# 10183308/popsift

Measured on AMD Instinct MI355X. Metric: Mpix/s SIFT extract on 1920x1080 (keypoints+descriptors), higher is better.
Workload: dtype f32; 1 GPU; 1920x1080 u8 grayscale, default popsift::Config (2x upscale, 9 octaves, 3 levels, PopSift mode, loop descriptor, RootSift); distinct_images_per_gpu=16, contexts_per_gpu=3, images_per_launch=16

## Files before the change

### include/popsift_hip.h

```cpp
#ifndef POPSIFT_HIP_H
#define POPSIFT_HIP_H

#include <stddef.h>
#include <stdint.h>

#ifdef __cplusplus
extern "C" {
#endif

#define POPSIFT_HIP_MAX_OCTAVES 20
#define POPSIFT_HIP_MAX_LEVELS 12
#define POPSIFT_HIP_MAX_BATCH 16
#define POPSIFT_HIP_GAUSS_ALIGN 32
#define POPSIFT_HIP_ORI_MAX 4

typedef enum popsift_hip_status {
    POPSIFT_HIP_OK = 0,
    POPSIFT_HIP_ERR_INVALID = -1,
    POPSIFT_HIP_ERR_DEVICE = -2,
    POPSIFT_HIP_ERR_NO_DEVICE = -3,
    POPSIFT_HIP_ERR_OOM = -4,
    POPSIFT_HIP_ERR_STATE = -5,
    POPSIFT_HIP_ERR_TOO_SMALL = -6
} popsift_hip_status;
// ... 189 lines not shown
    int32_t reserved;
} popsift_hip_match_opts;
typedef struct popsift_hip_pair {
    int32_t l, r;
    float   dist_best, dist_second;
} popsift_hip_pair;
void popsift_hip_default_match_opts(popsift_hip_match_opts* opts);
int  popsift_hip_match_pairs(const popsift_hip_devfeatures* l, const popsift_hip_devfeatures* r,
                             const popsift_hip_match_opts* opts, popsift_hip_pair* pairs, size_t cap, int* n_pairs);

typedef struct popsift_hip_bytefeatures popsift_hip_bytefeatures;
int popsift_hip_bytefeatures_from_host(int device, const uint8_t* desc, int n_descriptors, popsift_hip_bytefeatures** out);
int popsift_hip_bytefeatures_from_set(const popsift_hip_devfeatures* f, popsift_hip_bytefeatures** out);
int popsift_hip_clone_results_u8(popsift_hip_ctx* ctx, int k, popsift_hip_bytefeatures** out);
int popsift_hip_bytefeatures_free(popsift_hip_bytefeatures* f);
int popsift_hip_bytefeatures_info(const popsift_hip_bytefeatures* f, int* device, int* n_descriptors);
int popsift_hip_bytefeatures_download(const popsift_hip_bytefeatures* f, uint8_t* desc, int32_t* rev);
int popsift_hip_match_bytes(const popsift_hip_bytefeatures* l, const popsift_hip_bytefeatures* r, popsift_hip_match* out);
int popsift_hip_match_pairs_bytes(const popsift_hip_bytefeatures* l, const popsift_hip_bytefeatures* r,
                                  const popsift_hip_match_opts* opts, popsift_hip_pair* pairs, size_t cap, int* n_pairs);

int popsift_hip_get_report(const popsift_hip_ctx* ctx, popsift_hip_report* rep);
int popsift_hip_set_profile(popsift_hip_ctx* ctx, int profile);

int popsift_hip_octave_dims(const popsift_hip_ctx* ctx, int octave, int* w, int* h);
int popsift_hip_download_plane(popsift_hip_ctx* ctx, int octave, int kind, int level, float* out);
int popsift_hip_upload_plane(popsift_hip_ctx* ctx, int octave, int kind, int level, const float* in);
int popsift_hip_download_extrema(popsift_hip_ctx* ctx, popsift_hip_extremum* out, size_t cap, int* n);
int popsift_hip_rerun_keypoint_stages(popsift_hip_ctx* ctx);
enum { POPSIFT_HIP_DEBUG_DET_QCAP = 1, POPSIFT_HIP_DEBUG_CAND_CAP = 2, POPSIFT_HIP_DEBUG_OHIST_CAP = 3,
       POPSIFT_HIP_DEBUG_FAIL_ALLOC = 4, POPSIFT_HIP_DEBUG_DESC_ROWS = 5,
       POPSIFT_HIP_DEBUG_KP_WAVES = 7, POPSIFT_HIP_DEBUG_BLUR_PATH = 8, POPSIFT_HIP_DEBUG_BLUR_SEG = 9,
       POPSIFT_HIP_DEBUG_PYR_TAIL = 10, POPSIFT_HIP_DEBUG_DIRECT_PATH = 11,
       POPSIFT_HIP_DEBUG_DESC_CAP = 12, POPSIFT_HIP_DEBUG_SCALE_PATH = 13 };
int popsift_hip_debug_set(popsift_hip_ctx* ctx, int what, int value);

#ifdef __cplusplus
}
#endif
#endif
```

### popsift_amd/_capi.py

```python
import ctypes as C
import os

import numpy as np

_HERE = os.path.dirname(os.path.abspath(__file__))
LIB_PATH = os.environ.get("POPSIFT_HIP_LIB") or os.path.join(_HERE, "libpopsift_hip.so")

MAX_OCTAVES = 20
ORI_MAX = 4

OK = 0
ERR_INVALID, ERR_DEVICE, ERR_NO_DEVICE, ERR_OOM, ERR_STATE, ERR_TOO_SMALL = -1, -2, -3, -4, -5, -6

SIFT_POPSIFT, SIFT_OPENCV, SIFT_VLFEAT = 0, 1, 2
GAUSS_VLFEAT_COMPUTE, GAUSS_VLFEAT_RELATIVE, GAUSS_VLFEAT_RELATIVE_ALL = 0, 1, 2
GAUSS_OPENCV_COMPUTE, GAUSS_FIXED9, GAUSS_FIXED15 = 3, 4, 5
DESC_LOOP, DESC_ILOOP, DESC_GRID, DESC_IGRID, DESC_NOTILE = 0, 1, 2, 3, 4
NORM_ROOTSIFT, NORM_CLASSIC = 0, 1
SCALE_DEFAULT, SCALE_DIRECT = 0, 1


class Params(C.Structure):
    _fields_ = [
        ("octaves", C.c_int32), ("levels", C.c_int32), ("sigma", C.c_float),
# ... 94 lines not shown
    ("popsift_hip_devfeatures_free", C.c_int, [_vp]),
    ("popsift_hip_devfeatures_info", C.c_int, [_vp, _ip, _ip, _ip]),
    ("popsift_hip_devfeatures_ptrs", C.c_int, [_vp, C.POINTER(_vp), C.POINTER(_vp), C.POINTER(_vp)]),
    ("popsift_hip_devfeatures_alloc", C.c_int, [C.c_int, C.c_int, C.c_int, C.POINTER(_vp)]),
    ("popsift_hip_devfeatures_from_host", C.c_int, [C.c_int, _vp, C.c_int, C.POINTER(_vp)]),
    ("popsift_hip_devfeatures_download", C.c_int, [_vp, _vp, _vp]),
    ("popsift_hip_devfeatures_download_u8", C.c_int, [_vp, _vp]),
    ("popsift_hip_match_sets", C.c_int, [_vp, _vp, _vp]),
    ("popsift_hip_match_set_path", C.c_int, [C.c_int]),
    ("popsift_hip_default_match_opts", None, [C.POINTER(MatchOpts)]),
    ("popsift_hip_match_pairs", C.c_int, [_vp, _vp, C.POINTER(MatchOpts), _vp, C.c_size_t, _ip]),
    ("popsift_hip_bytefeatures_from_host", C.c_int, [C.c_int, _vp, C.c_int, C.POINTER(_vp)]),
    ("popsift_hip_bytefeatures_from_set", C.c_int, [_vp, C.POINTER(_vp)]),
    ("popsift_hip_clone_results_u8", C.c_int, [_vp, C.c_int, C.POINTER(_vp)]),
    ("popsift_hip_bytefeatures_free", C.c_int, [_vp]),
    ("popsift_hip_bytefeatures_info", C.c_int, [_vp, _ip, _ip]),
    ("popsift_hip_bytefeatures_download", C.c_int, [_vp, _vp, _vp]),
    ("popsift_hip_match_bytes", C.c_int, [_vp, _vp, _vp]),
    ("popsift_hip_match_pairs_bytes", C.c_int, [_vp, _vp, C.POINTER(MatchOpts), _vp, C.c_size_t, _ip]),
    ("popsift_hip_get_report", C.c_int, [_vp, C.POINTER(Report)]),
    ("popsift_hip_set_profile", C.c_int, [_vp, C.c_int]),
    ("popsift_hip_octave_dims", C.c_int, [_vp, C.c_int, _ip, _ip]),
    ("popsift_hip_download_plane", C.c_int, [_vp, C.c_int, C.c_int, C.c_int, _vp]),
    ("popsift_hip_upload_plane", C.c_int, [_vp, C.c_int, C.c_int, C.c_int, _vp]),
    ("popsift_hip_download_extrema", C.c_int, [_vp, _vp, C.c_size_t, _ip]),
    ("popsift_hip_rerun_keypoint_stages", C.c_int, [_vp]),
    ("popsift_hip_debug_set", C.c_int, [_vp, C.c_int, C.c_int]),
]
MATCH_AUTO, MATCH_EXACT, MATCH_SCREEN = 0, 1, 2
STAGES = ("pyramid", "detect", "refine", "orientation", "scan", "descriptor")
DEBUG_DET_QCAP, DEBUG_CAND_CAP, DEBUG_OHIST_CAP, DEBUG_FAIL_ALLOC, DEBUG_DESC_ROWS, DEBUG_KP_WAVES = 1, 2, 3, 4, 5, 7
DEBUG_BLUR_PATH, DEBUG_BLUR_SEG, DEBUG_PYR_TAIL, DEBUG_DIRECT_PATH, DEBUG_DESC_CAP = 8, 9, 10, 11, 12
DEBUG_SCALE_PATH = 13
MAX_BATCH = 16
IMG_HOST_U8, IMG_HOST_F32, IMG_DEV_U8, IMG_DEV_F32, IMG_PINNED_U8, IMG_PINNED_F32 = range(6)

_lib = None


def _desc_type(fmt):
    if fmt == "f32":
        return np.float32
    if fmt == "u8":
        return np.uint8
    raise ValueError("fmt: 'f32' or 'u8', got %r" % (fmt,))


def quantize_u8(desc):
    d = np.asarray(desc, np.float32)
    with np.errstate(invalid="ignore"):
        pos = d > 0
        t = np.trunc(d)
        r = np.where(np.abs(d - t) >= np.float32(0.5), t + np.float32(1.0), t)
        r = np.where(d >= np.float32(255.0), np.float32(255.0), r)
        r = np.where(pos, r, np.float32(0.0))
    return r.astype(np.uint8)


class PopsiftHipError(RuntimeError):
    def __init__(self, status, where, detail=""):
        self.status = status
        msg = "%s failed: %d (%s)" % (where, status, lib().popsift_hip_strerror(status).decode())
        if detail:
            msg += ": " + detail
        super().__init__(msg)

# ... 448 lines not shown
```

### popsift_amd/csrc/ctx.hip

```cpp
#include <hip/hip_runtime.h>

#include <algorithm>
#include <atomic>
#include <cmath>
#include <cstdarg>
#include <cstddef>
#include <cstdio>
#include <cstdlib>
#include <cstring>
#include <new>
#include <type_traits>
#include <vector>

#include "devfeatures.h"
#include "kernels.h"
#include "sift_types.h"
#include "trace.h"

using namespace popsift_hip;

namespace {

constexpr int PITCH_ALIGN = 64;
constexpr int PROFILE_REPS = 4;
// ... 72 lines not shown
};

struct popsift_hip_ctx {
    int                device = 0;
    popsift_hip_params p{};
    int                levels = 3, L = 6;
    GaussRows<POPSIFT_HIP_MAX_LEVELS> tab{};
    GaussRows<POPSIFT_HIP_MAX_LEVELS> abs0{};
    float*             d_abs0 = nullptr;
    int                direct_path = 0;
    GaussRows<POPSIFT_HIP_MAX_OCTAVES> dd{};
    float*             d_dd = nullptr;
    int                scale_path = 0;
    SiftConsts         sc{};
    hipStream_t        stream = nullptr;
    hipEvent_t         ev_begin = nullptr, ev_end = nullptr;
    hipEvent_t         ev_stage[POPSIFT_HIP_STAGE_COUNT + 1] = {};

    int  in_w = 0, in_h = 0;
    int  frozen_octaves = -1;
    bool have_image = false, finished = false;
    bool batch_ok = false;
    int  nb = 1;
    bool describe = false;
    int  ori_given = 0;
    int  frames_max = 0;

    ImageSlot slot[PS_MAX_BATCH];
    BatchDesc bd{};
    PyrDesc   pd{};
    int       kp_waves = 65536;
    int       det_qcap = 1 << 30;
    int       desc_rows = 1 << 30;
    BlurTune  blur_tune{0, 0};
    int       pyr_tail = 0;
    int       cand_cap_init = 1 << 20;
    bool      cand_cap_user = false;
    int       ohist_cap_init = 0;
    int       desc_cap_init = 0;
    size_t    ext_cap = 0;
    int       cand_cap = 0, desc_cap = 0;
    size_t    ohist_cap = 0;
    hipStream_t copy_stream = nullptr;
    hipEvent_t  ev_u8 = nullptr;
    bool     copy_pending = false;
    unsigned long submit_seq = 0, copy_seq = 0;
    Counters* d_ct = nullptr;
    Counters* h_ct = nullptr;
    PyrDesc*  d_pd = nullptr;
    PyrDesc*  h_pd = nullptr;
    int       n_feat[PS_MAX_BATCH] = {}, n_desc[PS_MAX_BATCH] = {};

    int                    fail_alloc_in = 0;
    int                    profile = 0;
    std::vector<EventPair> blur_events;
    size_t                 blur_events_used = 0;
    popsift_hip_report     rep{};

    char err[256] = {0};
};

namespace {

int fail(popsift_hip_ctx* c, int code, const char* fmt, ...)
{
    if (c) {
// ... 78 lines not shown
    auto& a0 = c->abs0;
    memset(&a0, 0, sizeof(a0));
    if (p.gauss_mode == POPSIFT_HIP_GAUSS_VLFEAT_RELATIVE_ALL) {
        for (int lvl = 0; lvl < c->L; lvl++) {
            const float sigmaS = sigma0 * powf(2.0f, (float)lvl / (float)levels);
            a0.sigma[lvl] = sqrtf(fabsf(sigmaS * sigmaS - initial_blur * initial_blur));
        }
        compute_filter_rows(a0, p.gauss_mode);
    }
    auto& dd = c->dd;
    memset(&dd, 0, sizeof(dd));
    for (int oct = 0; oct < POPSIFT_HIP_MAX_OCTAVES; oct++) {
        const float oct_sigma = ldexpf(sigma0, oct);
        const float b = sqrtf(fabsf(oct_sigma * oct_sigma - initial_blur * initial_blur));
        dd.sigma[oct] = ldexpf(b, -oct);
    }
    compute_filter_rows(dd, p.gauss_mode);
    SiftConsts& sc = c->sc;
    sc.sigma0 = sigma0;
    sc.sigma_k = powf(2.0f, 1.0f / levels);
    sc.edge_limit = p.edge_limit;
    sc.threshold = p.threshold * 0.5f * 255.0f / levels;
    sc.max_extrema = p.max_extrema;
    sc.norm_multi = p.norm_multi;
    sc.norm_mode = p.norm_mode;
    sc.sift_mode = p.sift_mode;
    sc.grid_size = p.filter_grid_size > 0 ? p.filter_grid_size : 1;
    sc.up_fac_int = (int)p.upscale_factor;
    sc.desc_mode = p.desc_mode;
    sc.filter_max = p.filter_max_extrema;
    sc.filter_mode = p.filter_sorting;
    sc.det_qcap = c->det_qcap;
    sc.desc_rows = c->desc_rows;
}

void plan_dims(const popsift_hip_ctx* c, int w, int h, int octaves_cfg, int* n_oct, int* bw, int* bh)
{
    const float scaleFactor = 1.0f / powf(2.0f, -c->p.upscale_factor);
    int         oct = octaves_cfg;
    if (oct < 0) oct = std::max(int(floorf(logf((float)std::min(w, h)) / logf(2.0f)) - 3.0f + scaleFactor), 1);
    oct = std::min(oct, PS_MAX_OCT);
    *n_oct = oct;
    *bw = (int)ceilf(w * scaleFactor);
    *bh = (int)ceilf(h * scaleFactor);
}

hipError_t ctx_malloc(popsift_hip_ctx* c, void** p, size_t bytes)
{
    if (c->fail_alloc_in > 0 && --c->fail_alloc_in == 0) {
        *p = nullptr;
        return hipErrorOutOfMemory;
    }
    return hipMalloc(p, bytes);
}

template <class T, size_t PER>
int grow(popsift_hip_ctx* c, DevBuf<T, PER>& b, size_t need)
{
    if (need <= b.cap) return 0;
    HIP_TRY(c, b.release());
    HIP_TRY(c, ctx_malloc(c, (void**)&b.p, need * PER * sizeof(T)));
    b.cap = need;
    return 0;
}

void refresh_caps(popsift_hip_ctx* c)
// ... 1847 lines not shown
    switch (what) {
    case POPSIFT_HIP_DEBUG_DET_QCAP:
        c->det_qcap = c->sc.det_qcap = std::max(value, 0);
        return POPSIFT_HIP_OK;
    case POPSIFT_HIP_DEBUG_CAND_CAP:
        c->cand_cap_init = std::max(value, DET_SUBQ);
        c->cand_cap_user = true;
        return POPSIFT_HIP_OK;
    case POPSIFT_HIP_DEBUG_OHIST_CAP:
        c->ohist_cap_init = std::max(value, 1);
        return POPSIFT_HIP_OK;
    case POPSIFT_HIP_DEBUG_DESC_CAP:
        c->desc_cap_init = std::max(value, 0);
        return POPSIFT_HIP_OK;
    case POPSIFT_HIP_DEBUG_FAIL_ALLOC:
        c->fail_alloc_in = std::max(value, 0);
        return POPSIFT_HIP_OK;
    case POPSIFT_HIP_DEBUG_KP_WAVES:
        c->kp_waves = std::min(std::max(value / 32 * 32, 32), 1 << 20);
        return POPSIFT_HIP_OK;
    case POPSIFT_HIP_DEBUG_BLUR_PATH:
        if (value < 0 || value > 2) return fail(c, POPSIFT_HIP_ERR_INVALID, "BLUR_PATH: 0, 1 or 2");
        c->blur_tune.path = value;
        return POPSIFT_HIP_OK;
    case POPSIFT_HIP_DEBUG_BLUR_SEG:
        c->blur_tune.seg_rows = std::max(value, 0);
        return POPSIFT_HIP_OK;
    case POPSIFT_HIP_DEBUG_PYR_TAIL:
        c->pyr_tail = value;
        return POPSIFT_HIP_OK;
    case POPSIFT_HIP_DEBUG_DESC_ROWS:
        c->desc_rows = c->sc.desc_rows = std::max(value, 4);
        return POPSIFT_HIP_OK;
    case POPSIFT_HIP_DEBUG_DIRECT_PATH:
        if (value < 0 || value > 1) return fail(c, POPSIFT_HIP_ERR_INVALID, "DIRECT_PATH: 0 or 1");
        c->direct_path = value;
        return POPSIFT_HIP_OK;
    case POPSIFT_HIP_DEBUG_SCALE_PATH:
        if (value < 0 || value > 1) return fail(c, POPSIFT_HIP_ERR_INVALID, "SCALE_PATH: 0 or 1");
        c->scale_path = value;
        return POPSIFT_HIP_OK;
    }
    return fail(c, POPSIFT_HIP_ERR_INVALID, "unknown debug switch %d", what);
}

int popsift_hip_rerun_keypoint_stages(popsift_hip_ctx* c)
{
    if (!c) return POPSIFT_HIP_ERR_INVALID;
    if (!c->have_image || !c->batch_ok) return fail(c, POPSIFT_HIP_ERR_STATE, "no image submitted");
    HIP_TRY(c, hipSetDevice(c->device));
    HIP_TRY(c, hipStreamSynchronize(c->stream));
    if (int rc = drain_copy(c)) return rc;
    c->blur_events_used = 0;
    HIP_TRY(c, hipEventRecord(c->ev_begin, c->stream));
    if (int rc = c->describe ? enqueue_describe_stages(c) : enqueue_keypoint_stages(c)) return rc;
    HIP_TRY(c, hipEventRecord(c->ev_end, c->stream));
    c->finished = false;
    for (ImageSlot& sl : c->slot) sl.moved = false;
    return POPSIFT_HIP_OK;
}

}
```

### popsift_amd/csrc/keypoint.hip

```cpp
#include <hip/hip_runtime.h>

#include "kernels.h"
#include "sift_types.h"

namespace popsift_hip {
namespace {

constexpr float F_PI = 3.14159265358979323846f;
constexpr float F_PI2 = 2.0f * 3.14159265358979323846f;
constexpr float            ORI_WINFACTOR = 1.5f;
constexpr float            DESC_MAGNIFY = 3.0f;

typedef unsigned long long fix64;
__device__ __forceinline__ fix64 to_fix(float w) { return (fix64)(unsigned int)(w * 1048576.0f); }
__device__ __forceinline__ float from_fix(fix64 v) { return (float)((double)v * (1.0 / 1048576.0)); }


__device__ __forceinline__ void wave_lds_sync()
{
    __builtin_amdgcn_fence(__ATOMIC_SEQ_CST, "wavefront");
    __builtin_amdgcn_wave_barrier();
}

__device__ __forceinline__ int wave_incl_scan(int v)
// ... 167 lines not shown
    const float ax = fabsf(x), ay = fabsf(y);
    const float mx = fmaxf(fmaxf(ax, ay), 1e-30f), mn = fminf(ax, ay);
    const float r = mn * __builtin_amdgcn_rcpf(mx);
    const float s = r * r;
    float       p = fmaf(-0.01492126751691103f, s, 0.06703268736600876f);
    p = fmaf(p, s, -0.14823880791664124f);
    p = fmaf(p, s, 0.24642325937747955f);
    p = fmaf(p, s, -0.42350852489471436f);
    p = fmaf(p, s, 1.2732105255126953f);
    return octants(p * r, x, y, ax, ay);
}

__device__ __forceinline__ float atan2_bins9(float y, float x)
{
    const float ax = fabsf(x), ay = fabsf(y);
    const float mx = fmaxf(fmaxf(ax, ay), 1e-30f), mn = fminf(ax, ay);
    const float r = mn * __builtin_amdgcn_rcpf(mx);
    const float s = r * r;
    float       p = fmaf(0.026540832594037056f, s, -0.1084246039390564f);
    p = fmaf(p, s, 0.22938621044158936f);
    p = fmaf(p, s, -0.4205572307109833f);
    p = fmaf(p, s, 1.2730693817138672f);
    return octants(p * r, x, y, ax, ay);
}

typedef float v2f __attribute__((ext_vector_type(2)));
typedef __attribute__((address_space(3))) fix64 lds_fix64;
typedef __attribute__((address_space(3))) unsigned int lds_u32;

#ifndef KP_NW
#define KP_NW 1
#endif
constexpr int ORI_COPIES = 4;

__global__ __launch_bounds__(64 * KP_NW) void k_orientation(const PyrDesc* __restrict__ pdp, BatchDesc bd, SiftConsts sc,
                                                     int filtered, int hist_cap)
{
    const float* __restrict__   arena = bd.s[blockIdx.y].arena;
    Counters* __restrict__      ct = bd.s[blockIdx.y].ct;
    const InitExt* __restrict__ iext = filtered ? bd.s[blockIdx.y].iext2 : bd.s[blockIdx.y].iext;
    float* __restrict__         ohist = bd.s[blockIdx.y].ohist;
    const int n_oct = pdp->n_oct, L = pdp->L;
    constexpr int    NB = PS_ORI_NBINS + 2;
    __shared__ fix64 s_hist[KP_NW][ORI_COPIES][NB];
    const int        wave = threadIdx.x >> 6, lane = threadIdx.x & 63;
    fix64*           hall = &s_hist[wave][0][0];
    fix64*           hist = s_hist[wave][lane & (ORI_COPIES - 1)];

    __shared__ int ps[PS_MAX_OCT + 1];
    if (threadIdx.x == 0) ext_prefix(ct, sc, n_oct, ps);
    __syncthreads();
    const int total = min(ps[n_oct], hist_cap);

    for (XcdSlice sl = xcd_slice<KP_NW>(); sl.more(total); sl.s += sl.step) {
        const int g = sl.index();
        if (g >= total) continue;
        int o = 0;
        while (o + 1 < n_oct && g >= ps[o + 1]) o++;
        o = uniform(o);
        const InitExt  ie = iext[(size_t)o * sc.max_extrema + (g - uniform(ps[o]))];
        const OctDesc* od = &pdp->o[o];
        const int      w = uniform(od->w), h = uniform(od->h), pitch = uniform(od->pitch);
        const int      lvl = uniform(min(max(ie.lpos, 0), L - 1));
        const float*   layer = arena + uniform64(od->data_off + lvl * od->plane_stride);

        for (int k = lane; k < ORI_COPIES * NB; k += 64) hall[k] = 0ull;
        wave_lds_sync();

        const float x = uniformf(ie.xpos), y = uniformf(ie.ypos), sig = uniformf(ie.sigma);
        const float sigw = ORI_WINFACTOR * sig;
        const int   rad = (int)roundf(3.0f * sigw);
        const float factor2 = (-0.5f / (sigw * sigw)) * 1.4426950408889634f;
        const int   sq_thres = rad * rad;
        const int   xmin = max(1, (int)roundf(x) - rad);
        const int   xmax = min(w - 2, (int)roundf(x) + rad);
        const int   ymin = max(1, (int)roundf(y) - rad);
        const int   ymax = min(h - 2, (int)roundf(y) + rad);
        const int   wx = xmax - xmin + 1;
        const int   hy = ymax - ymin + 1;
#ifdef ORI_PROBE_NOLOOP
        const int   loops = 0;
#else
        const int   loops = (wx > 0 && hy > 0) ? wx * hy : 0;
#endif
        const float inv_wx = __builtin_amdgcn_rcpf((float)max(wx, 1));
        const float wxf = (float)wx, xminf = (float)xmin, yminf = (float)ymin, pitch4f = (float)(4 * pitch);
        const float* corner = layer + (size_t)(ymin * pitch + xmin);

        auto coord = [&](int i, float& fx, float& fy, unsigned int& off) {
            const float fi = (float)i;
            const float frow = floorf((fi + 0.5f) * inv_wx);
            const float fcol = fmaf(-frow, wxf, fi);
            fx = fcol + xminf;
            fy = frow + yminf;
            off = (unsigned int)fmaf(frow, pitch4f, fcol * 4.0f);
        };
        auto bin = [&](float fx, float fy, float gdx, float gdy, bool live) {
            const float dx = fx - x;
            const float dy = fy - y;
            const float sq_dist = truncf(dx * dx + dy * dy);
            if (live && sq_dist <= (float)sq_thres) {
                const float wfix = __builtin_amdgcn_sqrtf(fmaf(gdx, gdx, gdy * gdy)) * __builtin_amdgcn_exp2f(fmaf(sq_dist, factor2, 20.0f));
                float fb = fmaf(atan2_bins(gdy, gdx), (float)PS_ORI_NBINS / 8.0f, (float)PS_ORI_NBINS / 2.0f);
                if (fabsf((fb - floorf(fb)) - 0.5f) < 1e-4f) fb = (float)PS_ORI_NBINS * (atan2_acc(gdy, gdx) + F_PI) / F_PI2;
                int bidx;
                asm("v_cvt_rpi_i32_f32 %0, %1" : "=v"(bidx) : "v"(fb));
                atomicAdd(&hist[bidx], (fix64)(unsigned int)wfix);
            }
        };
        float        xa = 0.0f, ya = 0.0f, xb = 0.0f, yb = 0.0f;
        unsigned int oa = 0, ob = 0;
        float        a0 = 0.0f, a1 = 0.0f, a2 = 0.0f, a3 = 0.0f, b0 = 0.0f, b1 = 0.0f, b2 = 0.0f, b3 = 0.0f;
        const Taps   taps(corner, pitch);
        if (loops > 0) {
            coord(min(lane, loops - 1), xa, ya, oa);
            taps.load_b(oa, a0, a1, a2, a3);
        }
        for (int i = lane; i < loops; i += 128) {
            coord(min(i + 64, loops - 1), xb, yb, ob);
            taps.load_b(ob, b0, b1, b2, b3);
            bin(xa, ya, a0 - a1, a2 - a3, true);
            coord(min(i + 128, loops - 1), xa, ya, oa);
            taps.load_b(oa, a0, a1, a2, a3);
            bin(xb, yb, b0 - b1, b2 - b3, i + 64 < loops);
        }
        wave_lds_sync();

        if (lane < PS_ORI_NBINS) {
            fix64 acc = 0ull;
#pragma unroll
            for (int k = 0; k < ORI_COPIES; k++) acc += hall[k * NB + lane] + (lane == 0 ? hall[k * NB + PS_ORI_NBINS] : 0ull);
            ohist[(size_t)g * PS_ORI_NBINS + lane] = from_fix(acc);
        }
        wave_lds_sync();
    }
}

__device__ __forceinline__ float quad_from_prev(float v)
{
    return __int_as_float(__builtin_amdgcn_update_dpp(0, __float_as_int(v), 0x93, 0xf, 0xf, false));
}
__device__ __forceinline__ float quad_from_next(float v)
{
    return __int_as_float(__builtin_amdgcn_update_dpp(0, __float_as_int(v), 0x39, 0xf, 0xf, false));
}
template <int CTRL>
__device__ __forceinline__ int quad_xchg(int v)
{
    return __builtin_amdgcn_update_dpp(0, v, CTRL, 0xf, 0xf, false);
}
__device__ __forceinline__ float div3(float x)
{
    const float r = 0.333333343267440796f;
    const float q = x * r;
    return fmaf(fmaf(-3.0f, q, x), r, q);
}

// ... 249 lines not shown
                    float sn, cs;
                    sincos_cr(e.orientation[q], sn, cs);
                    rot[idx + q] = make_float2(cs, sn);
                    if (drec) drec[idx + q] = make_desc_rec(pdp, e, e.orientation[q], cs, sn);
                }
            }
            feats[g] = f;
            for (int o = 0; o < n_oct; o++)
                if (g == s_ps[o] && s_ps[o + 1] > s_ps[o]) ct->ori_ps[o] = idx;
        }
    }
    if (tid == 0 && chunk == nb - 1) {
        int last = chunk_offset;
        for (int k = 0; k < SCAN_SUB && (chunk * SCAN_SUB + k) * SCAN_LCHUNK < total; k++) last += partial[chunk * SCAN_SUB + k];
        ct->ori_total = last;
        ct->ext_total = total;
        for (int o = 0; o < PS_MAX_OCT; o++) {
            ct->ext_ct[o] = (o < n_oct) ? min(ct->ext_ct[o], sc.max_extrema) : 0;
            ct->ext_ps[o] = s_ps[o];
        }
    }
    __syncthreads();
    }
}


#ifndef DESC_NCOPY
#define DESC_NCOPY 4
#endif
constexpr int DESC_COPIES = DESC_NCOPY;
constexpr int DESC_RS = 36;
constexpr int DESC_CS = 3 * DESC_RS + 32;
constexpr int DESC_MAXROWS = 128;

__global__ __launch_bounds__(64 * KP_NW, 8) void k_descriptor(BatchDesc bd, SiftConsts sc, int desc_cap)
{
    const float* __restrict__   arena = bd.s[blockIdx.y].arena;
    const Counters* __restrict__ ct = bd.s[blockIdx.y].ct;
    const DescRec* __restrict__ drec = bd.s[blockIdx.y].drec;
    float* __restrict__         desc = bd.s[blockIdx.y].desc;
    constexpr int ROW_WORDS = (DESC_MAXROWS + 1 + 3) & ~3;
    static_assert(ROW_WORDS * 4 >= 352, "cell (-1, -1) of copy 0 stays inside the wave's LDS");
    __shared__ __attribute__((aligned(16))) unsigned int s_lds[KP_NW][ROW_WORDS + 2 * DESC_COPIES * DESC_CS];
    const int     lane = threadIdx.x & 63, wave = threadIdx.x >> 6;
    const int     cpy = lane & (DESC_COPIES - 1);
    unsigned int* rinfo = s_lds[wave];
    fix64*        hall = (fix64*)(s_lds[wave] + ROW_WORDS);
    const unsigned int rbase32 = (unsigned int)(size_t)(lds_u32*)rinfo;
    const float        hbasef = (float)(unsigned int)(size_t)(lds_fix64*)(hall + cpy * DESC_CS);
    const float        cpy8f = (float)(cpy << 3);
    const int     total = min(ct->ori_total, desc_cap);
    const int     maxrows = min(max(sc.desc_rows, 4), DESC_MAXROWS);

    for (XcdSlice sl = xcd_slice<KP_NW>(); sl.more(total); sl.s += sl.step) {
        const int d = sl.index();
        if (d >= total) continue;
        typedef unsigned int u4 __attribute__((ext_vector_type(4)));
        const u4*          rp = reinterpret_cast<const u4*>(drec + d);
        const u4           q0 = rp[0], q1 = rp[1], q2 = rp[2];
        const float        x = uniformf(__uint_as_float(q0.x)), y = uniformf(__uint_as_float(q0.y));
        const float        crsbp = uniformf(__uint_as_float(q0.z)), srsbp = uniformf(__uint_as_float(q0.w));
        const float        ang_bins = uniformf(__uint_as_float(q1.x));
        const float        inv_c = uniformf(__uint_as_float(q1.y)), inv_s = uniformf(__uint_as_float(q2.w));
        const int          pmin = uniform((int)q1.z), pmax = uniform((int)q1.w);
        const unsigned int misc = (unsigned int)uniform((int)q2.z);
        const int          pitch = (int)(misc & 0xffffu), fbits = (int)((misc >> 16) & 0xffu);
        const float*       layer = arena + uniform64((long long)(((unsigned long long)q2.y << 32) | q2.x));

        {
            u4 zero;
            asm volatile("v_mov_b32 %0, 0\n\tv_mov_b32 %1, 0\n\tv_mov_b32 %2, 0\n\tv_mov_b32 %3, 0"
                         : "=v"(zero.x), "=v"(zero.y), "=v"(zero.z), "=v"(zero.w));
            constexpr int CLEAR16 = DESC_COPIES * DESC_CS / 2;
            static_assert(DESC_COPIES * DESC_CS % 2 == 0, "whole 16-byte pieces");
            u4*           h16 = reinterpret_cast<u4*>(hall);
#pragma unroll
            for (int k = 0; k < (CLEAR16 + 63) / 64; k++)
                if (lane + 64 * k < CLEAR16) h16[lane + 64 * k] = zero;
        }

        if (misc & (1u << 24)) {
            const int   xmin = (int)(short)(pmin & 0xffff), ymin0 = pmin >> 16;
            const int   xmax = (int)(short)(pmax & 0xffff), ymax = pmax >> 16;
            const int   wx = xmax - xmin + 1;
            const int   hy_all = ymax - ymin0 + 1;
            const float ffbits = (float)fbits;

            for (int rb = 0; rb < hy_all && wx > 0; rb += maxrows) {
            const int   ymin = ymin0 + rb;
            const int   hy = min(hy_all - rb, maxrows);

            int T = 0, grow = 0;
            {
                int         carry = 0;
                for (int r0 = 0; r0 < hy; r0 += 64) {
                    const int r = r0 + lane;
                    int       len = 0, jlo = xmin;
                    if (r < hy) {
                        const float dy = (float)(ymin + r) - y;
                        const float a = srsbp * dy, b = crsbp * dy;
                        float       lo = -1e30f, hi = 1e30f;
                        bool        ok = true;
                        if (inv_c != 0.0f) {
                            const float t0 = (-2.5f - a) * inv_c, t1 = (2.5f - a) * inv_c;
                            lo = fminf(t0, t1);
                            hi = fmaxf(t0, t1);
                        } else {
                            ok = fabsf(a) < 2.5f;
                        }
                        if (inv_s != 0.0f) {
                            const float t0 = (b - 2.5f) * inv_s, t1 = (b + 2.5f) * inv_s;
                            lo = fmaxf(lo, fminf(t0, t1));
                            hi = fminf(hi, fmaxf(t0, t1));
                        } else {
                            ok = ok && (fabsf(b) < 2.5f);
                        }
                        jlo = max(xmin, (int)floorf(x + lo - 1e-3f) + 1);
                        const int jhi = min(xmax, (int)ceilf(x + hi + 1e-3f) - 1);
                        len = ok ? max(jhi - jlo + 1, 0) : 0;
                        if (len == 0) jlo = xmin;
                    }
                    const int incl = wave_incl_scan(len);
                    const int start = carry + incl - len;
                    if (r < hy) rinfo[r] = (unsigned int)start | ((unsigned int)(start - (jlo - xmin)) << 16);
                    const unsigned long long live = __ballot(len > 0);
                    if (carry == 0 && live != 0ull) grow = r0 + __ffsll((long long)live) - 1;
                    carry += __builtin_amdgcn_readlane(incl, 63);
                }
                T = carry;
                if (lane == 0) {
                    rinfo[hy] = (unsigned int)T | 0x7fff0000u;
                    rinfo[hy + 1] = 0xffffu;
                }
            }
            wave_lds_sync();

#ifdef DESC_PROBE_NOLOOP
            const int   steps = 0;
#else
            const int   steps = (T + 63) >> 6;
#endif
            unsigned int rp = rbase32 + 4u * (unsigned int)grow;
            float        fr = (float)(rb + grow);
            unsigned int cur = 0;
            unsigned int nxt = 0x7fff0000u | 0xffffu;
            if (T > 0) {
                cur = rinfo[grow];
                nxt = rinfo[grow + 1];
            }

            const float  ox = (float)xmin - x, oy = (float)ymin0 - y;
            const float  u0 = fmaf(crsbp, ox, srsbp * oy), v0 = fmaf(crsbp, oy, -srsbp * ox);
            const float* corner = layer + (size_t)(ymin0 * pitch + xmin);
            const float  pitch4f = (float)(4 * pitch);

            auto coord = [&](int i, unsigned int& off, float& u, float& v) {
                while (i >= (int)(nxt & 0xffffu)) {
                    fr += 1.0f;
                    rp += 4u;
                    cur = nxt;
                    nxt = *(lds_u32*)(size_t)(rp + 4u);
                }
                const float fc = (float)(i - ((int)cur >> 16));
                u = fmaf(crsbp, fc, fmaf(srsbp, fr, u0));
                v = fmaf(crsbp, fr, fmaf(-srsbp, fc, v0));
                asm("v_cvt_u32_f32 %0, %1" : "=v"(off) : "v"(fmaf(fr, pitch4f, fc * 4.0f)));
            };
            unsigned int probe_acc = 0u;
            auto bin = [&](float u, float v, float gx, float gy) {
                if (fabsf(u) < 2.5f && fabsf(v) < 2.5f) {
                    const float  mod = __builtin_amdgcn_sqrtf(fmaf(gx, gx, gy * gy));
                    const float  wm = __builtin_amdgcn_exp2f(fmaf(-0.18033688011112042f, fmaf(u, u, v * v), ffbits)) * mod;
                    const float tth = atan2_bins9(gy, gx) - ang_bins;
                    const float ffo = floorf(tth);
                    const float do0 = tth - ffo;

                    const float tu = u + 1.5f, tv = v + 1.5f;
                    const float fcx = floorf(tu), fcy = floorf(tv);
                    const float fx = tu - fcx, fy = tv - fcy;
                    const float wx0 = 1.0f - fx, wy0 = (1.0f - fy) * wm, wy1 = fy * wm;
                    const float w0 = 1.0f - do0;
                    const unsigned int s0 = (unsigned int)(int)fmaf(fcx, 32.0f, fmaf(ffo, 8.0f, cpy8f)) & 56u;
                    const unsigned int cb = (unsigned int)(int)fmaf(fcy, (float)(DESC_RS * 8), fmaf(fcx, 64.0f, hbasef));
                    const unsigned int e0 = cb + s0;
                    const unsigned int e1 = (s0 ^ 32u) + cb;
                    const bool x0 = tu >= 0.0f, x1 = tu < 3.0f, y0 = tv >= 0.0f, y1 = tv < 3.0f;
#ifdef DESC_PROBE_NOATOMIC
#define PS_CELL_ADD(ADDR, LO, HI) probe_acc ^= (LO) ^ (HI) ^ (ADDR);
#else
#define PS_CELL_ADD(ADDR, LO, HI)                                                                             \
    __hip_atomic_fetch_add((lds_fix64*)(size_t)(ADDR), ((fix64)(HI) << 32) | (fix64)(LO), __ATOMIC_RELAXED,    \
                           __HIP_MEMORY_SCOPE_WORKGROUP);
#endif
#define PS_CELL(ADDR, WGT)                                                                                     \
    {                                                                                                          \
        const float        wgt = (WGT);                                                                        \
        const unsigned int lo = __float_as_uint(fmaf(w0, wgt, 8388608.0f)) & 0x7fffffu;                        \
        const unsigned int hi = __float_as_uint(fmaf(do0, wgt, 8388608.0f)) & 0x7fffffu;                       \
        PS_CELL_ADD(ADDR, lo, hi)                                                                              \
    }
                    if (y0) {
                        if (x0) PS_CELL(e0, wy0 * wx0)
                        if (x1) PS_CELL(e1 + 64u, wy0 * fx)
                    }
                    if (y1) {
                        if (x0) PS_CELL(e0 + DESC_RS * 8u, wy1 * wx0)
                        if (x1) PS_CELL(e1 + DESC_RS * 8u + 64u, wy1 * fx)
                    }
#undef PS_CELL
#undef PS_CELL_ADD
                }
            };
            unsigned int off_a = 0, off_b = 0;
            float u_a = 3.0f, v_a = 3.0f, a0 = 0.0f, a1 = 0.0f, a2 = 0.0f, a3 = 0.0f;
            float u_b = 3.0f, v_b = 3.0f, b0 = 0.0f, b1 = 0.0f, b2 = 0.0f, b3 = 0.0f;
            const Taps taps(corner, pitch);
#ifdef DESC_PROBE_NOLOAD
#define PS_TAPS(OFF, A0, A1, A2, A3) { A0 = __uint_as_float(OFF) * 1e-9f; A1 = u0; A2 = v0; A3 = __uint_as_float((OFF) ^ 0x3f800000u); }
#else
#define PS_TAPS(OFF, A0, A1, A2, A3) taps.load_b(OFF, A0, A1, A2, A3);
#endif
            if (T > 0) {
                coord(lane, off_a, u_a, v_a);
                PS_TAPS(off_a, a0, a1, a2, a3)
            }
            int t = steps, i = lane;
            for (; t > 2; t -= 2, i += 128) {
                coord(i + 64, off_b, u_b, v_b);
                PS_TAPS(off_b, b0, b1, b2, b3)
                bin(u_a, v_a, a0 - a1, a2 - a3);
                coord(i + 128, off_a, u_a, v_a);
                PS_TAPS(off_a, a0, a1, a2, a3)
                bin(u_b, v_b, b0 - b1, b2 - b3);
            }
            if (t == 2) {
                coord(i + 64, off_b, u_b, v_b);
                PS_TAPS(off_b, b0, b1, b2, b3)
            }
            if (t > 0) bin(u_a, v_a, a0 - a1, a2 - a3);
            if (t == 2) bin(u_b, v_b, b0 - b1, b2 - b3);
            if (probe_acc == 0x12345u) desc[(size_t)d * 128 + lane] = 1.0f;
            wave_lds_sync();
            }
        }
        wave_lds_sync();

        fix64 a0 = 0ull, a1 = 0ull;
        {
            const int b = lane & 7, ix = (lane >> 3) & 3, iyl = lane >> 5;
#pragma unroll
            for (int k = 0; k < DESC_COPIES; k++) {
                const int sl = (b + k + ((ix & 1) << 2)) & 7, sh = (b + 7 + k + ((ix & 1) << 2)) & 7;
                const int c0 = k * DESC_CS + iyl * DESC_RS + ix * 8;
                const int c1 = k * DESC_CS + (iyl + 2) * DESC_RS + ix * 8;
                a0 += (hall[c0 + sl] & 0xffffffffull) + (hall[c0 + sh] >> 32);
                a1 += (hall[c1 + sl] & 0xffffffffull) + (hall[c1 + sh] >> 32);
            }
        }
        const float inv_scale = scalbnf(1.0f, -fbits);
        float       v0 = (float)a0 * inv_scale, v1 = (float)a1 * inv_scale;

        if (sc.norm_mode == POPSIFT_HIP_NORM_ROOTSIFT) {
            float sum = v0 + v1;
            sum = wave_allsum(sum);
            const float rs = __builtin_amdgcn_rcpf(sum);
            v0 = scalbnf(__builtin_amdgcn_sqrtf(v0 * rs), sc.norm_multi);
            v1 = scalbnf(__builtin_amdgcn_sqrtf(v1 * rs), sc.norm_multi);
        } else {
            float sq = v0 * v0 + v1 * v1;
// ... 351 lines not shown
```

### popsift_amd/csrc/sift_types.h

```cpp
#pragma once
#include <stdint.h>

#include <hip/hip_vector_types.h>

#include "../../include/popsift_hip.h"

#define PS_MAX_OCT POPSIFT_HIP_MAX_OCTAVES
#define PS_MAX_PLANES (POPSIFT_HIP_MAX_LEVELS + 3)
#define PS_GA POPSIFT_HIP_GAUSS_ALIGN
#define PS_ORI_NBINS 36

struct OctDesc {
    float*  data;
    float*  dog;
    int64_t data_off;
    int64_t dog_off;
    int64_t plane_stride;
    int     w, h, pitch;
    int     tile_begin;
};

struct PyrDesc {
    int     n_oct;
    int     levels;
    int     L;
    int     total_tiles;
    int     dog_fly;
    int     pad_;
    OctDesc o[PS_MAX_OCT];
};

struct SiftConsts {
    float sigma0, sigma_k, edge_limit, threshold;
    int   max_extrema, norm_multi, norm_mode, sift_mode;
    int   grid_size;
    int   up_fac_int;
    int   desc_mode;
    int   det_qcap;
    int   filter_max;
    int   filter_mode;
    int   desc_rows;
};

struct InitExt {
    float xpos, ypos;
    int   lpos;
    float sigma;
    int   cell;
};

struct Ext {
    float xpos, ypos;
    int   lpos;
    float sigma;
    int   octave;
    int   num_ori;
    int   idx_ori;
    float orientation[POPSIFT_HIP_ORI_MAX];
};

struct DescRec {
    float        x, y;
    float        crsbp, srsbp;
    float        ang_bins;
    float        inv_c;
    unsigned int xymin, xymax;
    unsigned int off_lo, off_hi;
    unsigned int misc;
    float        inv_s;
};

static_assert(sizeof(DescRec) == 48, "three 16-byte loads");

struct Counters {
// ... 65 lines not shown
```

Baseline: 3616 Mpix/s.

## Iterate only pixels inside the circular window in orientation histogram

```diff
diff --git a/include/popsift_hip.h b/include/popsift_hip.h
--- a/include/popsift_hip.h
+++ b/include/popsift_hip.h
@@ -245,7 +245,7 @@
        POPSIFT_HIP_DEBUG_FAIL_ALLOC = 4, POPSIFT_HIP_DEBUG_DESC_ROWS = 5,
        POPSIFT_HIP_DEBUG_KP_WAVES = 7, POPSIFT_HIP_DEBUG_BLUR_PATH = 8, POPSIFT_HIP_DEBUG_BLUR_SEG = 9,
        POPSIFT_HIP_DEBUG_PYR_TAIL = 10, POPSIFT_HIP_DEBUG_DIRECT_PATH = 11,
-       POPSIFT_HIP_DEBUG_DESC_CAP = 12, POPSIFT_HIP_DEBUG_SCALE_PATH = 13 };
+       POPSIFT_HIP_DEBUG_DESC_CAP = 12, POPSIFT_HIP_DEBUG_SCALE_PATH = 13, POPSIFT_HIP_DEBUG_ORI_ROWS = 14 };
 int popsift_hip_debug_set(popsift_hip_ctx* ctx, int what, int value);
 
 #ifdef __cplusplus
diff --git a/popsift_amd/_capi.py b/popsift_amd/_capi.py
--- a/popsift_amd/_capi.py
+++ b/popsift_amd/_capi.py
@@ -150,6 +150,7 @@
 DEBUG_DET_QCAP, DEBUG_CAND_CAP, DEBUG_OHIST_CAP, DEBUG_FAIL_ALLOC, DEBUG_DESC_ROWS, DEBUG_KP_WAVES = 1, 2, 3, 4, 5, 7
 DEBUG_BLUR_PATH, DEBUG_BLUR_SEG, DEBUG_PYR_TAIL, DEBUG_DIRECT_PATH, DEBUG_DESC_CAP = 8, 9, 10, 11, 12
 DEBUG_SCALE_PATH = 13
+DEBUG_ORI_ROWS = 14
 MAX_BATCH = 16
 IMG_HOST_U8, IMG_HOST_F32, IMG_DEV_U8, IMG_DEV_F32, IMG_PINNED_U8, IMG_PINNED_F32 = range(6)
 
diff --git a/popsift_amd/csrc/ctx.hip b/popsift_amd/csrc/ctx.hip
--- a/popsift_amd/csrc/ctx.hip
+++ b/popsift_amd/csrc/ctx.hip
@@ -128,6 +128,7 @@
     int       kp_waves = 65536;
     int       det_qcap = 1 << 30;
     int       desc_rows = 1 << 30;
+    int       ori_rows = 1 << 30;
     BlurTune  blur_tune{0, 0};
     int       pyr_tail = 0;
     int       cand_cap_init = 1 << 20;
@@ -272,6 +273,7 @@
     sc.filter_mode = p.filter_sorting;
     sc.det_qcap = c->det_qcap;
     sc.desc_rows = c->desc_rows;
+    sc.ori_rows = c->ori_rows;
 }
 
 void plan_dims(const popsift_hip_ctx* c, int w, int h, int octaves_cfg, int* n_oct, int* bw, int* bh)
@@ -2185,6 +2187,9 @@
     case POPSIFT_HIP_DEBUG_DESC_ROWS:
         c->desc_rows = c->sc.desc_rows = std::max(value, 4);
         return POPSIFT_HIP_OK;
+    case POPSIFT_HIP_DEBUG_ORI_ROWS:
+        c->ori_rows = c->sc.ori_rows = std::max(value, 1);
+        return POPSIFT_HIP_OK;
     case POPSIFT_HIP_DEBUG_DIRECT_PATH:
         if (value < 0 || value > 1) return fail(c, POPSIFT_HIP_ERR_INVALID, "DIRECT_PATH: 0 or 1");
         c->direct_path = value;
diff --git a/popsift_amd/csrc/keypoint.hip b/popsift_amd/csrc/keypoint.hip
--- a/popsift_amd/csrc/keypoint.hip
+++ b/popsift_amd/csrc/keypoint.hip
@@ -223,6 +223,7 @@
 #define KP_NW 1
 #endif
 constexpr int ORI_COPIES = 4;
+constexpr int ORI_MAXROWS = 64;
 
 __global__ __launch_bounds__(64 * KP_NW) void k_orientation(const PyrDesc* __restrict__ pdp, BatchDesc bd, SiftConsts sc,
                                                      int filtered, int hist_cap)
@@ -237,6 +238,10 @@
     const int        wave = threadIdx.x >> 6, lane = threadIdx.x & 63;
     fix64*           hall = &s_hist[wave][0][0];
     fix64*           hist = s_hist[wave][lane & (ORI_COPIES - 1)];
+    __shared__ unsigned int s_rows[KP_NW][ORI_MAXROWS + 2];
+    unsigned int*           rinfo = s_rows[wave];
+    const unsigned int      rbase32 = (unsigned int)(size_t)(lds_u32*)rinfo;
+    const int               maxrows = min(max(sc.ori_rows, 1), ORI_MAXROWS);
 
     __shared__ int ps[PS_MAX_OCT + 1];
     if (threadIdx.x == 0) ext_prefix(ct, sc, n_oct, ps);
@@ -263,34 +268,23 @@
         const int   rad = (int)roundf(3.0f * sigw);
         const float factor2 = (-0.5f / (sigw * sigw)) * 1.4426950408889634f;
         const int   sq_thres = rad * rad;
-        const int   xmin = max(1, (int)roundf(x) - rad);
-        const int   xmax = min(w - 2, (int)roundf(x) + rad);
-        const int   ymin = max(1, (int)roundf(y) - rad);
+        const int   xr = (int)roundf(x);
+        const int   xmin = max(1, xr - rad);
+        const int   xmax = min(w - 2, xr + rad);
+        const int   ymin0 = max(1, (int)roundf(y) - rad);
         const int   ymax = min(h - 2, (int)roundf(y) + rad);
         const int   wx = xmax - xmin + 1;
-        const int   hy = ymax - ymin + 1;
-#ifdef ORI_PROBE_NOLOOP
-        const int   loops = 0;
-#else
-        const int   loops = (wx > 0 && hy > 0) ? wx * hy : 0;
-#endif
-        const float inv_wx = __builtin_amdgcn_rcpf((float)max(wx, 1));
-        const float wxf = (float)wx, xminf = (float)xmin, yminf = (float)ymin, pitch4f = (float)(4 * pitch);
-        const float* corner = layer + (size_t)(ymin * pitch + xmin);
-
-        auto coord = [&](int i, float& fx, float& fy, unsigned int& off) {
-            const float fi = (float)i;
-            const float frow = floorf((fi + 0.5f) * inv_wx);
-            const float fcol = fmaf(-frow, wxf, fi);
-            fx = fcol + xminf;
-            fy = frow + yminf;
-            off = (unsigned int)fmaf(frow, pitch4f, fcol * 4.0f);
-        };
-        auto bin = [&](float fx, float fy, float gdx, float gdy, bool live) {
+        const int   hy_all = ymax - ymin0 + 1;
+        const float xminf = (float)xmin, yminf = (float)ymin0, pitch4f = (float)(4 * pitch);
+        const float* corner = layer + (size_t)(ymin0 * pitch + xmin);
+        const float r1 = (float)(sq_thres + 1);
+        const float x0 = x - (float)xr;
+
+        auto bin = [&](float fx, float fy, float gdx, float gdy) {
             const float dx = fx - x;
             const float dy = fy - y;
             const float sq_dist = truncf(dx * dx + dy * dy);
-            if (live && sq_dist <= (float)sq_thres) {
+            if (sq_dist <= (float)sq_thres) {
                 const float wfix = __builtin_amdgcn_sqrtf(fmaf(gdx, gdx, gdy * gdy)) * __builtin_amdgcn_exp2f(fmaf(sq_dist, factor2, 20.0f));
                 float fb = fmaf(atan2_bins(gdy, gdx), (float)PS_ORI_NBINS / 8.0f, (float)PS_ORI_NBINS / 2.0f);
                 if (fabsf((fb - floorf(fb)) - 0.5f) < 1e-4f) fb = (float)PS_ORI_NBINS * (atan2_acc(gdy, gdx) + F_PI) / F_PI2;
@@ -299,21 +293,72 @@
                 atomicAdd(&hist[bidx], (fix64)(unsigned int)wfix);
             }
         };
-        float        xa = 0.0f, ya = 0.0f, xb = 0.0f, yb = 0.0f;
-        unsigned int oa = 0, ob = 0;
-        float        a0 = 0.0f, a1 = 0.0f, a2 = 0.0f, a3 = 0.0f, b0 = 0.0f, b1 = 0.0f, b2 = 0.0f, b3 = 0.0f;
-        const Taps   taps(corner, pitch);
-        if (loops > 0) {
-            coord(min(lane, loops - 1), xa, ya, oa);
-            taps.load_b(oa, a0, a1, a2, a3);
-        }
-        for (int i = lane; i < loops; i += 128) {
-            coord(min(i + 64, loops - 1), xb, yb, ob);
-            taps.load_b(ob, b0, b1, b2, b3);
-            bin(xa, ya, a0 - a1, a2 - a3, true);
-            coord(min(i + 128, loops - 1), xa, ya, oa);
-            taps.load_b(oa, a0, a1, a2, a3);
-            bin(xb, yb, b0 - b1, b2 - b3, i + 64 < loops);
+
+        for (int rb = 0; rb < hy_all && wx > 0; rb += maxrows) {
+            const int hy = min(hy_all - rb, maxrows);
+            int       len = 0, c0 = xmin;
+            if (lane < hy) {
+                const float dy = (float)(ymin0 + rb + lane) - y;
+                const float s = __builtin_amdgcn_sqrtf(fmaxf(r1 - dy * dy, 0.0f));
+                c0 = max(xmin, xr + (int)ceilf(x0 - s - 1e-3f));
+                const int c1 = min(xmax, xr + (int)floorf(x0 + s + 1e-3f));
+                len = max(c1 - c0 + 1, 0);
+                if (len == 0) c0 = xmin;
+            }
+            const int incl = wave_incl_scan(len);
+            const int start = incl - len;
+            if (lane < hy) rinfo[lane] = (unsigned int)(start & 0xffff) | ((unsigned int)(start - (c0 - xmin)) << 16);
+            const int T = __builtin_amdgcn_readlane(incl, 63);
+            if (lane == 0) {
+                rinfo[hy] = (unsigned int)T | 0x7fff0000u;
+                rinfo[hy + 1] = 0xffffu;
+            }
+            wave_lds_sync();
+
+#ifdef ORI_PROBE_NOLOOP
+            const int steps = 0;
+#else
+            const int steps = (T + 63) >> 6;
+#endif
+            unsigned int rp = rbase32;
+            float        fr = (float)rb;
+            unsigned int cur = rinfo[0], nxt = rinfo[1];
+            auto coord = [&](int i, float& fx, float& fy, unsigned int& off) {
+                while (i >= (int)(nxt & 0xffffu)) {
+                    fr += 1.0f;
+                    rp += 4u;
+                    cur = nxt;
+                    nxt = *(lds_u32*)(size_t)(rp + 4u);
+                }
+                const float fc = (float)(i - ((int)cur >> 16));
+                fx = fc + xminf;
+                fy = fr + yminf;
+                asm("v_cvt_u32_f32 %0, %1" : "=v"(off) : "v"(fmaf(fr, pitch4f, fc * 4.0f)));
+            };
+            float        xa = 0.0f, ya = 0.0f, xb = 0.0f, yb = 0.0f;
+            unsigned int oa = 0, ob = 0;
+            float        a0 = 0.0f, a1 = 0.0f, a2 = 0.0f, a3 = 0.0f, b0 = 0.0f, b1 = 0.0f, b2 = 0.0f, b3 = 0.0f;
+            const Taps   taps(corner, pitch);
+            if (steps > 0) {
+                coord(lane, xa, ya, oa);
+                taps.load_b(oa, a0, a1, a2, a3);
+            }
+            int t = steps, i = lane;
+            for (; t > 2; t -= 2, i += 128) {
+                coord(i + 64, xb, yb, ob);
+                taps.load_b(ob, b0, b1, b2, b3);
+                bin(xa, ya, a0 - a1, a2 - a3);
+                coord(i + 128, xa, ya, oa);
+                taps.load_b(oa, a0, a1, a2, a3);
+                bin(xb, yb, b0 - b1, b2 - b3);
+            }
+            if (t == 2) {
+                coord(i + 64, xb, yb, ob);
+                taps.load_b(ob, b0, b1, b2, b3);
+            }
+            if (t > 0) bin(xa, ya, a0 - a1, a2 - a3);
+            if (t == 2) bin(xb, yb, b0 - b1, b2 - b3);
+            wave_lds_sync();
         }
         wave_lds_sync();
 
diff --git a/popsift_amd/csrc/sift_types.h b/popsift_amd/csrc/sift_types.h
--- a/popsift_amd/csrc/sift_types.h
+++ b/popsift_amd/csrc/sift_types.h
@@ -40,6 +40,7 @@
     int   filter_max;
     int   filter_mode;
     int   desc_rows;
+    int   ori_rows;
 };
 
 struct InitExt {
```

Measured after the change: 3645 Mpix/s (median of 6 runs). No clear change (+0.8%).

## Replace serial row-walk in descriptor with LDS bitmap and mbcnt row lookup

Applied to the files above, without the earlier changes.

```diff
diff --git a/include/popsift_hip.h b/include/popsift_hip.h
--- a/include/popsift_hip.h
+++ b/include/popsift_hip.h
@@ -245,7 +245,7 @@
        POPSIFT_HIP_DEBUG_FAIL_ALLOC = 4, POPSIFT_HIP_DEBUG_DESC_ROWS = 5,
        POPSIFT_HIP_DEBUG_KP_WAVES = 7, POPSIFT_HIP_DEBUG_BLUR_PATH = 8, POPSIFT_HIP_DEBUG_BLUR_SEG = 9,
        POPSIFT_HIP_DEBUG_PYR_TAIL = 10, POPSIFT_HIP_DEBUG_DIRECT_PATH = 11,
-       POPSIFT_HIP_DEBUG_DESC_CAP = 12, POPSIFT_HIP_DEBUG_SCALE_PATH = 13 };
+       POPSIFT_HIP_DEBUG_DESC_CAP = 12, POPSIFT_HIP_DEBUG_SCALE_PATH = 13, POPSIFT_HIP_DEBUG_DESC_POS = 14 };
 int popsift_hip_debug_set(popsift_hip_ctx* ctx, int what, int value);
 
 #ifdef __cplusplus
diff --git a/popsift_amd/_capi.py b/popsift_amd/_capi.py
--- a/popsift_amd/_capi.py
+++ b/popsift_amd/_capi.py
@@ -150,6 +150,7 @@
 DEBUG_DET_QCAP, DEBUG_CAND_CAP, DEBUG_OHIST_CAP, DEBUG_FAIL_ALLOC, DEBUG_DESC_ROWS, DEBUG_KP_WAVES = 1, 2, 3, 4, 5, 7
 DEBUG_BLUR_PATH, DEBUG_BLUR_SEG, DEBUG_PYR_TAIL, DEBUG_DIRECT_PATH, DEBUG_DESC_CAP = 8, 9, 10, 11, 12
 DEBUG_SCALE_PATH = 13
+DEBUG_DESC_POS = 14
 MAX_BATCH = 16
 IMG_HOST_U8, IMG_HOST_F32, IMG_DEV_U8, IMG_DEV_F32, IMG_PINNED_U8, IMG_PINNED_F32 = range(6)
 
diff --git a/popsift_amd/csrc/ctx.hip b/popsift_amd/csrc/ctx.hip
--- a/popsift_amd/csrc/ctx.hip
+++ b/popsift_amd/csrc/ctx.hip
@@ -128,6 +128,7 @@
     int       kp_waves = 65536;
     int       det_qcap = 1 << 30;
     int       desc_rows = 1 << 30;
+    int       desc_pos = 1 << 30;
     BlurTune  blur_tune{0, 0};
     int       pyr_tail = 0;
     int       cand_cap_init = 1 << 20;
@@ -272,6 +273,7 @@
     sc.filter_mode = p.filter_sorting;
     sc.det_qcap = c->det_qcap;
     sc.desc_rows = c->desc_rows;
+    sc.desc_pos = c->desc_pos;
 }
 
 void plan_dims(const popsift_hip_ctx* c, int w, int h, int octaves_cfg, int* n_oct, int* bw, int* bh)
@@ -2185,6 +2187,9 @@
     case POPSIFT_HIP_DEBUG_DESC_ROWS:
         c->desc_rows = c->sc.desc_rows = std::max(value, 4);
         return POPSIFT_HIP_OK;
+    case POPSIFT_HIP_DEBUG_DESC_POS:
+        c->desc_pos = c->sc.desc_pos = std::max(value, 64);
+        return POPSIFT_HIP_OK;
     case POPSIFT_HIP_DEBUG_DIRECT_PATH:
         if (value < 0 || value > 1) return fail(c, POPSIFT_HIP_ERR_INVALID, "DIRECT_PATH: 0 or 1");
         c->direct_path = value;
diff --git a/popsift_amd/csrc/keypoint.hip b/popsift_amd/csrc/keypoint.hip
--- a/popsift_amd/csrc/keypoint.hip
+++ b/popsift_amd/csrc/keypoint.hip
@@ -629,6 +629,8 @@
 constexpr int DESC_RS = 36;
 constexpr int DESC_CS = 3 * DESC_RS + 32;
 constexpr int DESC_MAXROWS = 128;
+constexpr int DESC_MAXPOS = 63 * 64;
+constexpr unsigned int DESC_ROW_NONE = 32767u;
 
 __global__ __launch_bounds__(64 * KP_NW, 8) void k_descriptor(BatchDesc bd, SiftConsts sc, int desc_cap)
 {
@@ -647,7 +649,8 @@
     const float        hbasef = (float)(unsigned int)(size_t)(lds_fix64*)(hall + cpy * DESC_CS);
     const float        cpy8f = (float)(cpy << 3);
     const int     total = min(ct->ori_total, desc_cap);
-    const int     maxrows = min(max(sc.desc_rows, 4), DESC_MAXROWS);
+    const int     maxrows_cfg = min(max(sc.desc_rows, 4), DESC_MAXROWS);
+    const int     maxpos = min(max(sc.desc_pos, 64), DESC_MAXPOS);
 
     for (XcdSlice sl = xcd_slice<KP_NW>(); sl.more(total); sl.s += sl.step) {
         const int d = sl.index();
@@ -683,13 +686,21 @@
             const int   hy_all = ymax - ymin0 + 1;
             const float ffbits = (float)fbits;
 
+            const int   maxrows = max(min(maxrows_cfg, maxpos / max(wx, 1)), 1);
             for (int rb = 0; rb < hy_all && wx > 0; rb += maxrows) {
             const int   ymin = ymin0 + rb;
             const int   hy = min(hy_all - rb, maxrows);
 
+            fix64 keep = 0ull;
+            if (rb > 0) {
+                keep = hall[lane];
+                hall[lane] = 0ull;
+            }
+            wave_lds_sync();
             int T = 0, grow = 0;
             {
                 int         carry = 0;
+                lds_u32*    bmw = (lds_u32*)(size_t)(lds_fix64*)hall;
                 for (int r0 = 0; r0 < hy; r0 += 64) {
                     const int r = r0 + lane;
                     int       len = 0, jlo = xmin;
@@ -719,17 +730,22 @@
                     }
                     const int incl = wave_incl_scan(len);
                     const int start = carry + incl - len;
-                    if (r < hy) rinfo[r] = (unsigned int)start | ((unsigned int)(start - (jlo - xmin)) << 16);
+                    if (r < hy) rinfo[r] = (len > 0) ? (unsigned int)(start - (jlo - xmin)) : DESC_ROW_NONE;
+                    if (len > 0) {
+                        const int p = start + len - 1;
+                        __hip_atomic_fetch_or(bmw + (p >> 5), 1u << (p & 31), __ATOMIC_RELAXED, __HIP_MEMORY_SCOPE_WORKGROUP);
+                    }
                     const unsigned long long live = __ballot(len > 0);
                     if (carry == 0 && live != 0ull) grow = r0 + __ffsll((long long)live) - 1;
                     carry += __builtin_amdgcn_readlane(incl, 63);
                 }
                 T = carry;
-                if (lane == 0) {
-                    rinfo[hy] = (unsigned int)T | 0x7fff0000u;
-                    rinfo[hy + 1] = 0xffffu;
-                }
+                if (lane == 0) rinfo[hy] = DESC_ROW_NONE;
             }
+            wave_lds_sync();
+            const fix64        bmq = hall[lane];
+            hall[lane] = keep;
+            const unsigned int bm_lo = (unsigned int)bmq, bm_hi = (unsigned int)(bmq >> 32);
             wave_lds_sync();
 
 #ifdef DESC_PROBE_NOLOOP
@@ -737,28 +753,38 @@
 #else
             const int   steps = (T + 63) >> 6;
 #endif
-            unsigned int rp = rbase32 + 4u * (unsigned int)grow;
-            float        fr = (float)(rb + grow);
-            unsigned int cur = 0;
-            unsigned int nxt = 0x7fff0000u | 0xffffu;
-            if (T > 0) {
-                cur = rinfo[grow];
-                nxt = rinfo[grow + 1];
-            }
+            int                rows_before = rb + grow;
+            const unsigned int rbase_rb = rbase32 - 4u * (unsigned int)rb;
+            float              fr_n = 0.0f;
+            unsigned int       cur_n = 0u;
+            auto row_at = [&](int k) {
+                const unsigned int wl = __builtin_amdgcn_readlane(bm_lo, k), wh = __builtin_amdgcn_readlane(bm_hi, k);
+#ifdef DESC_PROBE_ROWARITH
+                const unsigned int row = (unsigned int)(rb + min(grow + (64 * k + lane) / 37, hy - 1));
+#else
+                const unsigned int row = __builtin_amdgcn_mbcnt_hi(wh, __builtin_amdgcn_mbcnt_lo(wl, (unsigned int)rows_before));
+                rows_before += __builtin_popcount(wl) + __builtin_popcount(wh);
+#endif
+                fr_n = (float)row;
+                cur_n = *(lds_u32*)(size_t)(rbase_rb + 4u * row);
+            };
+            if (T > 0) row_at(0);
+            auto row_ready = [&]() { asm volatile("" : : "v"(cur_n) : "memory"); };
 
             const float  ox = (float)xmin - x, oy = (float)ymin0 - y;
             const float  u0 = fmaf(crsbp, ox, srsbp * oy), v0 = fmaf(crsbp, oy, -srsbp * ox);
             const float* corner = layer + (size_t)(ymin0 * pitch + xmin);
             const float  pitch4f = (float)(4 * pitch);
 
-            auto coord = [&](int i, unsigned int& off, float& u, float& v) {
-                while (i >= (int)(nxt & 0xffffu)) {
-                    fr += 1.0f;
-                    rp += 4u;
-                    cur = nxt;
-                    nxt = *(lds_u32*)(size_t)(rp + 4u);
-                }
-                const float fc = (float)(i - ((int)cur >> 16));
+            auto coord = [&](int k, unsigned int& off, float& u, float& v) {
+                const float        fr = fr_n;
+                const unsigned int cur = cur_n;
+                row_at(k + 1);
+#ifdef DESC_PROBE_ROWARITH
+                const float fc = (float)min(max(64 * k + lane - (int)cur, 0), wx - 1);
+#else
+                const float fc = (float)(64 * k + lane - (int)cur);
+#endif
                 u = fmaf(crsbp, fc, fmaf(srsbp, fr, u0));
                 v = fmaf(crsbp, fr, fmaf(-srsbp, fc, v0));
                 asm("v_cvt_u32_f32 %0, %1" : "=v"(off) : "v"(fmaf(fr, pitch4f, fc * 4.0f)));
@@ -818,20 +844,22 @@
 #define PS_TAPS(OFF, A0, A1, A2, A3) taps.load_b(OFF, A0, A1, A2, A3);
 #endif
             if (T > 0) {
-                coord(lane, off_a, u_a, v_a);
+                coord(0, off_a, u_a, v_a);
                 PS_TAPS(off_a, a0, a1, a2, a3)
             }
-            int t = steps, i = lane;
-            for (; t > 2; t -= 2, i += 128) {
-                coord(i + 64, off_b, u_b, v_b);
+            int t = steps, k = 0;
+            for (; t > 2; t -= 2, k += 2) {
+                coord(k + 1, off_b, u_b, v_b);
                 PS_TAPS(off_b, b0, b1, b2, b3)
+                row_ready();
                 bin(u_a, v_a, a0 - a1, a2 - a3);
-                coord(i + 128, off_a, u_a, v_a);
+                coord(k + 2, off_a, u_a, v_a);
                 PS_TAPS(off_a, a0, a1, a2, a3)
+                row_ready();
                 bin(u_b, v_b, b0 - b1, b2 - b3);
             }
             if (t == 2) {
-                coord(i + 64, off_b, u_b, v_b);
+                coord(k + 1, off_b, u_b, v_b);
                 PS_TAPS(off_b, b0, b1, b2, b3)
             }
             if (t > 0) bin(u_a, v_a, a0 - a1, a2 - a3);
diff --git a/popsift_amd/csrc/sift_types.h b/popsift_amd/csrc/sift_types.h
--- a/popsift_amd/csrc/sift_types.h
+++ b/popsift_amd/csrc/sift_types.h
@@ -40,6 +40,7 @@
     int   filter_max;
     int   filter_mode;
     int   desc_rows;
+    int   desc_pos;
 };
 
 struct InitExt {
```

New measurement: 3662 Mpix/s before, 3757 Mpix/s after (median of 6 runs). 2.6% higher.
